# rasd3/3D-Dual-Fusion

Hardware: AMD Instinct MI355X
Metric: nuScenes sweeps/sec (0.075 m voxel, ~60k pts) (higher is better)
Workload: dtype f32 (fp32-grade throughout: every matrix-core GEMM -- C>=32 sparse convs, neck / head convs, FFN, query linears, image projection, value GEMM -- takes its fp32 operands as fp16 hi+lo pairs, 22 significand bits, 3 MFMA products, fp32 accumulate: <= 4e-6 of scale against float64, the grade of the exac

## Files before the change

### 3d-dual-fusion_amd/csrc/headconv.hip

```cpp
#include "common.h"
#include <algorithm>

namespace df3d {

typedef float f32x4 __attribute__((ext_vector_type(4)));
typedef unsigned int u32x4 __attribute__((ext_vector_type(4)));

constexpr int HF_TILE = 8, HF_HALO = HF_TILE + 2, HF_HP = HF_HALO * HF_HALO, HF_C = 64, HF_KMAX = 4;
constexpr int HF_LD = HF_HP + 1;

struct HeadFinalArgs {
  const u32x4 *in;
  const float *w;
  const u32x4 *wp;
  const float *bias;
  const int32_t *cols;
  float *out;
  int ld, ldo, B, H, W, G, tiles_x, tiles_y, gpad;
};

DF3D_SPLIT_OVERFLOW_TU(headconv)

__global__ __launch_bounds__(256) void head_final_kernel(HeadFinalArgs a) {
  __shared__ float x[HF_C * HF_LD];
// ... 274 lines not shown
        const int dy = tap / 3, dx = tap - dy * 3;
        const float *xp = x + lane * HF_LD + dy * HF_HALO + dx;
        for (int p = 0; p < 64; ++p) {
          const float xv = xp[(p >> 3) * HF_HALO + (p & 7)];
          const f32x4 g4 = *(const f32x4 *)&go[p * HF_KMAX];
          acc[i][0] = fmaf(xv, g4[0], acc[i][0]);
          acc[i][1] = fmaf(xv, g4[1], acc[i][1]);
          acc[i][2] = fmaf(xv, g4[2], acc[i][2]);
          acc[i][3] = fmaf(xv, g4[3], acc[i][3]);
        }
      }
    }
  }
#pragma unroll
  for (int i = 0; i < 3; ++i) {
    const int tap = wave + 4 * i;
    if (tap < 9) {
      float *dst = a.gw + (((size_t)g * 9 + tap) * HF_C + lane) * HF_KMAX;
#pragma unroll
      for (int j = 0; j < HF_KMAX; ++j)
        if (j < k && acc[i][j] != 0.f) unsafeAtomicAdd(dst + j, acc[i][j]);
    }
  }
}

}

using namespace df3d;

extern "C" size_t df3d_head_final_packed_bytes(int groups) { return groups > 0 ? (size_t)groups * 6 * 128 * 16 : 0; }

extern "C" int df3d_head_final_pack(const float *weights, int groups, void *packed, void *stream_) {
  hipStream_t stream = (hipStream_t)stream_;
  DF3D_CHECK_ARG(weights && packed && groups >= 1, "head_final_pack: bad argument");
  hipLaunchKernelGGL(head_final_pack_kernel, dim3(groups * 6), dim3(64), 0, stream, weights, (u32x4 *)packed);
  DF3D_LAUNCH_CHECK();
  return DF3D_OK;
}

static int head_final_impl(const void *in_split, int in_channels, int batch, int H, int W, int groups, const float *weights,
                           const void *packed, const float *bias, const int32_t *out_cols, float *out, int out_channels,
                           void *stream_);

extern "C" int df3d_head_final_conv(const void *in_split, int in_channels, int batch, int H, int W, int groups,
                                    const float *weights, const float *bias, const int32_t *out_cols, float *out,
                                    int out_channels, void *stream_) {
// ... 53 lines not shown
                                             const int32_t *out_cols, float *grad_acts, float *grad_weights, void *stream_) {
  hipStream_t stream = (hipStream_t)stream_;
  DF3D_CHECK_ARG(grad_out && weights && out_cols && (grad_acts || grad_weights), "head_final_conv_backward: null argument");
  DF3D_CHECK_ARG(groups >= 1 && act_channels >= groups * HF_C && act_channels % 4 == 0,
                 "head_final_conv_backward: %d branches of 64 channels do not fit %d-channel rows", groups, act_channels);
  DF3D_CHECK_ARG(batch >= 1 && H >= 1 && W >= 1 && out_channels >= 1, "head_final_conv_backward: bad sizes");
  DF3D_CHECK_ARG(!grad_weights || acts, "head_final_conv_backward: the filter gradient needs the activations");
  HeadFinalBwdArgs a;
  a.m = acts, a.go = grad_out, a.w = weights, a.cols = out_cols, a.gm = grad_acts, a.gw = grad_weights;
  a.ldm = act_channels, a.ldo = out_channels, a.B = batch, a.H = H, a.W = W, a.G = groups;
  a.tiles_x = cdiv(W, HF_TILE), a.tiles_y = cdiv(H, HF_TILE);
  const int ntiles = batch * a.tiles_x * a.tiles_y;
  a.tiles_per_wg = 1;
  if (grad_acts)
    hipLaunchKernelGGL(head_final_bwd_data_kernel, dim3(ntiles, groups), dim3(256), 0, stream, a);
  if (grad_weights) {
    DF3D_HIP(hipMemsetAsync(grad_weights, 0, (size_t)groups * 9 * HF_C * HF_KMAX * sizeof(float), stream));
    a.tiles_per_wg = std::max(1, cdiv(ntiles, 64));
    hipLaunchKernelGGL(head_final_bwd_filter_kernel, dim3(cdiv(ntiles, a.tiles_per_wg), groups), dim3(256), 0, stream, a);
  }
  DF3D_LAUNCH_CHECK();
  return DF3D_OK;
}
```

### 3d-dual-fusion_amd/dualfusion/_lib.py

```python
import ctypes
import os

_HERE = os.path.dirname(os.path.abspath(__file__))
LIB_PATH = os.path.join(os.path.dirname(_HERE), "csrc", "libdf3d_hip.so")

c_int = ctypes.c_int
c_uint = ctypes.c_uint
c_longlong = ctypes.c_longlong
c_size_t = ctypes.c_size_t
c_float = ctypes.c_float
c_void_p = ctypes.c_void_p
c_ulonglong = ctypes.c_ulonglong
c_char_p = ctypes.c_char_p

SIGNATURES = {
    "df3d_version": (c_int, []),
    "df3d_last_error": (c_char_p, []),
    "df3d_device_count": (c_int, []),
    "df3d_device_arch": (c_int, [c_char_p, c_int]),
    "df3d_split_overflow": (c_int, [c_int, c_char_p, c_int]),
    "df3d_split_overflow_collect": (c_int, [c_void_p, c_int, c_void_p]),
    "df3d_split_overflow_units": (c_int, [c_char_p, c_int]),
    "df3d_hard_voxelize_workspace_bytes": (c_size_t, [c_int, c_int, c_int]),
    "df3d_hard_voxelize": (c_int, [c_void_p, c_int, c_int, c_void_p, c_void_p, c_int, c_int, c_int,
# ... 130 lines not shown
    "df3d_sparse_conv_grad_filters": (c_int, [c_void_p, c_int, c_int, c_void_p, c_int, c_int, c_void_p, c_int, c_void_p,
                                              c_void_p]),
    "df3d_conv_rows_split": (c_int, [c_void_p, c_int, c_int, c_int, c_int, c_void_p, c_int, c_int, c_int, c_void_p, c_int,
                                     c_void_p, c_void_p, c_void_p, c_int, c_void_p, c_int, c_void_p, c_void_p, c_void_p]),
    "df3d_conv_packed_weight_bytes3": (c_size_t, [c_int, c_int, c_int]),
    "df3d_conv_pack_weights3": (c_int, [c_void_p, c_int, c_int, c_int, c_int, c_void_p, c_void_p]),
    "df3d_split_rows3": (c_int, [c_void_p, ctypes.c_longlong, c_int, c_void_p, c_void_p]),
    "df3d_conv_rows_split3": (c_int, [c_void_p, c_int, c_int, c_int, c_int, c_void_p, c_int, c_int, c_int, c_void_p, c_int,
                                      c_void_p, c_void_p, c_void_p, c_void_p, c_int, c_void_p, c_int, c_void_p, c_void_p,
                                      c_void_p]),
    "df3d_boxes_bev_pairwise": (c_int, [c_void_p, c_int, c_void_p, c_int, c_int, c_void_p, c_void_p]),
    "df3d_nms_bev_workspace_bytes": (c_size_t, [c_int, c_int]),
    "df3d_nms_bev": (c_int, [c_void_p, c_void_p, c_int, c_int, c_float, c_int, c_int, c_void_p, c_void_p, c_void_p,
                             c_size_t, c_void_p]),
    "df3d_centerhead_predict_workspace_bytes": (c_size_t, [c_int, c_void_p]),
    "df3d_centerhead_predict": (c_int, [c_void_p, c_int, c_void_p, c_void_p, c_void_p, c_void_p, c_void_p, c_void_p,
                                        c_size_t, c_void_p]),
    "df3d_head_final_conv": (c_int, [c_void_p, c_int, c_int, c_int, c_int, c_int, c_void_p, c_void_p, c_void_p, c_void_p,
                                     c_int, c_void_p]),
    "df3d_head_final_packed_bytes": (c_size_t, [c_int]),
    "df3d_head_final_pack": (c_int, [c_void_p, c_int, c_void_p, c_void_p]),
    "df3d_head_final_conv_packed": (c_int, [c_void_p, c_int, c_int, c_int, c_int, c_int, c_void_p, c_void_p, c_void_p,
                                            c_void_p, c_int, c_void_p]),
    "df3d_head_final_conv_backward": (c_int, [c_void_p, c_int, c_void_p, c_int, c_int, c_int, c_int, c_int, c_void_p, c_void_p,
                                              c_void_p, c_void_p, c_void_p]),
    "df3d_centerhead_loss_workspace_bytes": (c_size_t, [c_int, c_int, c_int, c_int]),
    "df3d_centerhead_loss": (c_int, [c_void_p, c_void_p, c_int, c_int, c_int, c_int, c_int, c_int, c_void_p, c_int, c_float,
                                     c_void_p, c_void_p, c_size_t, c_void_p]),
    "df3d_centerhead_loss_grad": (c_int, [c_void_p, c_void_p, c_void_p, c_int, c_int, c_int, c_int, c_int, c_int, c_void_p, c_int, c_float,
                                     c_void_p, c_void_p, c_size_t, c_void_p]),
    "df3d_heatmap_proposals_workspace_bytes": (c_size_t, [c_int, c_int, c_int, c_int]),
    "df3d_heatmap_proposals": (c_int, [c_void_p, c_int, c_int, c_int, c_int, c_int, c_int, c_uint, c_int, c_void_p, c_int,
                                       c_int, c_void_p, c_void_p, c_void_p, c_void_p, c_void_p, c_void_p, c_void_p,
                                       c_void_p, c_size_t, c_void_p]),
    "df3d_transfusion_decode": (c_int, [c_void_p, c_void_p, c_void_p, c_int, c_int, c_int, c_void_p, c_void_p, c_void_p,
                                        c_void_p, c_void_p, c_void_p]),
    "df3d_furthest_point_sample_with_dist": (c_int, [c_void_p, c_int, c_int, c_int, c_void_p, c_void_p, c_void_p]),
    "df3d_group_points_grad": (c_int, [c_void_p, c_void_p, c_int, c_int, c_int, c_int, c_int, c_void_p, c_void_p]),
    "df3d_gather_points_grad": (c_int, [c_void_p, c_void_p, c_int, c_int, c_int, c_int, c_void_p, c_void_p]),
    "df3d_rows_linear_packed_bytes": (c_size_t, [c_int, c_int]),
    "df3d_rows_linear": (c_int, [c_void_p, c_void_p, c_void_p, c_longlong, c_int, c_void_p, c_int, c_int, c_void_p, c_void_p, c_int,
                                 c_int, c_void_p, c_int, c_int, c_void_p, c_void_p, c_void_p, c_float, c_void_p]),
    "df3d_voxel_image_sample": (c_int, [c_void_p, c_int, c_int, c_float, c_void_p, c_void_p, c_void_p, c_void_p, c_void_p, c_int, c_int,
                                        c_int, c_int, c_int, c_float, c_float, c_void_p, c_void_p, c_void_p, c_void_p, c_void_p,
                                        c_void_p]),
    "df3d_backbone_inputs_ready": (c_int, [c_void_p]),
# ... 133 lines not shown
```

### 3d-dual-fusion_amd/dualfusion/apitimer.py

```python
import ctypes

from . import _lib

_NO_STREAM = ("df3d_version", "df3d_last_error", "df3d_device_count", "df3d_device_arch", "df3d_timing_", "df3d_ffn_set_precision",
              "df3d_conv_tile_count", "df3d_bn_rows_supported", "df3d_bn_rows_scratch_doubles", "df3d_debug_")
CONV_ENTRIES = ("df3d_sparse_conv_fused", "df3d_sparse_conv_grouped", "df3d_sparse_conv_fused_tiled", "df3d_sparse_conv_split", "df3d_sparse_conv_bf16",
                "df3d_conv_rows_split", "df3d_backbone_run")


def _ops_stream():
    from . import ops
    return ops._stream()


def _ival(a):
    if isinstance(a, bool):
        return int(a)
    if isinstance(a, int):
        return a
    if isinstance(a, (ctypes.c_int, ctypes.c_longlong, ctypes.c_size_t, ctypes.c_uint)):
        return int(a.value)
    if isinstance(a, float):
        return a
    if isinstance(a, ctypes.c_float):
# ... 101 lines not shown
    return B * ncam * max_ne * (C + Ci + 5) * 4, 0, "hbm", "gather of %d x %d query slots: %d voxel + %d image channels" % (B * ncam, max_ne, C, Ci)


def _rows(elems_in, elems_out, what):
    return (elems_in + elems_out) * 4, 0, "hbm", what


MODELS = {
    "df3d_hard_voxelize": lambda a, x: (20 * a[1] + a[6] * 0, 0, "hbm", "hash + scan + gather of %d points (bytes completed by the caller with M * 36)" % a[1]),
    "df3d_hard_voxelize_batched": lambda a, x: (20 * a[1], 0, "hbm", "hash + scan + gather of %d points (bytes completed by the caller with M * 36)" % a[1]),
    "df3d_ms_deform_attn_fused": lambda a, x: _msda(a, 4),
    "df3d_ms_deform_attn_fused_bf16": lambda a, x: _msda(a, 2),
    "df3d_ffn_fused_jobs": lambda a, x: _ffn(a, x),
    "df3d_imgproj_split": lambda a, x: _imgproj(a),
    "df3d_value_fold_gemm": lambda a, x: _value_gemm(a, 4),
    "df3d_value_fold_gemm_bf16": lambda a, x: _value_gemm(a, 2),
    "df3d_assemble_queries2": lambda a, x: _assemble(a),
    "df3d_sparse_to_dense": lambda a, x: (a[2] * a[3] * 4, 0, "hbm", "dense(): %d rows x %d channels scattered (+ the zero fill of the dense tensor)" % (a[2], a[3])),
    "df3d_sparse_to_dense_rows": lambda a, x: (a[2] * a[3] * 4, 0, "hbm", "dense() as pixel rows: %d rows x %d channels (+ the zero fill)" % (a[2], a[3])),
    "df3d_head_final_conv": lambda a, x: (a[2] * a[3] * a[4] * (a[1] * 4 + a[10] * 4), 2 * a[2] * a[3] * a[4] * a[5] * 9 * 64 * 4, "hbm",
                                          "final 3x3 convs of %d head branches on %d pixels" % (a[5], a[2] * a[3] * a[4])),
    "df3d_head_final_conv_packed": lambda a, x: (a[2] * a[3] * a[4] * (a[1] * 4 + a[10] * 4), 2 * a[2] * a[3] * a[4] * a[5] * 9 * 64 * 4, "hbm",
                                                 "final 3x3 convs of %d head branches on %d pixels (taps as matrix-core columns)" % (a[5], a[2] * a[3] * a[4])),
    "df3d_split_rows": lambda a, x: _rows(a[1] * a[2], a[1] * a[2], "fp32 rows -> split rows (%d x %d)" % (a[1], a[2])),
    "df3d_actr_prep": lambda a, x: _rows(3 * a[3] * a[4], 2 * a[3] * a[4], "query + position sums (%d rows)" % a[3]),
    "df3d_add_layernorm": lambda a, x: _rows(2 * a[5] * a[6], a[5] * a[6], "add + LayerNorm (%d rows)" % a[5]),
    "df3d_add_layernorm_split": lambda a, x: _rows(2 * a[5] * a[6], 2 * a[5] * a[6], "add + LayerNorm + split rows (%d rows)" % a[5]),
    "df3d_bigate_sum": lambda a, x: _rows(2 * a[6] * a[7], 2 * a[6] * a[7], "bidirectional gate (%d rows)" % a[6]),
    "df3d_rows_groupnorm": lambda a, x: _rows(2 * a[1] * a[2] * a[3], a[1] * a[2] * a[3], "GroupNorm over query rows (two passes)"),
    "df3d_fusion_writeback": lambda a, x: _rows(a[5] * a[6] + a[7] * a[8] * a[6], a[5] * a[6], "additive write-back of %d voxels" % a[5]),
    "df3d_rows_linear": lambda a, x: (a[3] * (a[4] + a[6]) * 4 + a[4] * a[6] * 4, 2 * a[3] * a[4] * a[6], "hbm",
                                      "query linear %d -> %d over %d rows (one input stream counted)" % (a[4], a[6], a[3])),
    "df3d_lt_layer": lambda a, x: (2 * a[1] * a[2] * a[3] * 4, a[1] * a[2] * 2 * (3 * 64 * 64 + 64 * 64 + 2 * 128 * 64 + 2 * 32 * 64), "hbm",
                                   "LocalTransformer layer over %d groups of %d tokens" % (a[2], a[1])),
    "df3d_lt_layer_gather": lambda a, x: (2 * 32 * a[3] * 64 * 4 + 32 * a[3] * 20, 32 * a[3] * 2 * (3 * 64 * 64 + 64 * 64 + 2 * 128 * 64 + 2 * 32 * 64 + 32 * 64), "hbm",
                                          "LocalTransformer layer with gather + positional MLP, %d groups" % a[3]),
    "df3d_lt_layer_scatter": lambda a, x: (2 * 32 * a[1] * 64 * 4 + 32 * a[1] * 8, 32 * a[1] * 2 * (3 * 64 * 64 + 64 * 64 + 2 * 128 * 64 + 2 * 32 * 64), "hbm",
                                           "LocalTransformer layer with winner write-back, %d groups" % a[1]),
    "df3d_voxel_image_sample": lambda a, x: (a[1] * (16 + a[9] * 4 * 5), 0, "hbm", "point-fusion sampling of %d voxels x %d channels" % (a[1], a[9])),
    "df3d_project_voxels": lambda a, x: (a[1] * 16 + a[1] * a[3] * (8 + 1 + 12 + 4), 0, "hbm", "projection of %d voxels into %d cameras" % (a[1], a[3])),
    "df3d_query_slots": lambda a, x: (a[2] * a[4] * 5 + a[2] * 16, 0, "hbm", "per-camera query slots of %d voxels" % a[2]),
}
RULEBOOK_ENTRIES = ("df3d_grid_build", "df3d_subm_neighbors", "df3d_conv_out_indices", "df3d_conv_neighbors",
                    "df3d_conv_transpose_out_indices", "df3d_conv_transpose_neighbors", "df3d_conv2d_neighbors", "df3d_nbr_to_pairs",
                    "df3d_pairs_to_nbr", "df3d_invert_neighbors")

# ... 30 lines not shown
```

### 3d-dual-fusion_amd/dualfusion/heads.py

```python
import copy
import os

import torch
from torch import nn

from . import ops as _ops
from .registry import HEADS


def _clamped_sigmoid(x):
    return torch.clamp(x.sigmoid_(), min=1e-4, max=1 - 1e-4)


def _transpose_and_gather_feat(feat, ind):
    feat = feat.permute(0, 2, 3, 1).contiguous()
    feat = feat.view(feat.size(0), -1, feat.size(3))
    return feat.gather(1, ind.unsqueeze(2).expand(ind.size(0), ind.size(1), feat.size(2)))


def reg_loss(output, mask, ind, target):
    pred = _transpose_and_gather_feat(output, ind)
    mask = mask.float().unsqueeze(2)
    loss = torch.nn.functional.l1_loss(pred * mask, target * mask, reduction='none')
    loss = loss / (mask.sum() + 1e-4)
# ... 69 lines not shown
        go = grad_out.contiguous().float()
        g_a, g_w = _ops.head_final_conv_backward(acts, go, B, H, W, w4d.shape[0], w4d, cols)
        sums = torch.cat([go.sum(0), go.new_zeros(1)])
        c = cols.long()
        j = torch.arange(4, device=go.device)
        idx = torch.where(j[None, :] < c[:, 1:2], c[:, 0:1] + j[None, :], torch.full_like(c[:, 0:1], go.shape[1]))
        return g_a, g_w, sums[idx], None, None, None, None, None


class _PermuteGather(torch.autograd.Function):

    @staticmethod
    def forward(ctx, src, idx, inv):
        ctx.save_for_backward(inv)
        return src.index_select(0, idx)

    @staticmethod
    @torch.autograd.function.once_differentiable
    def backward(ctx, grad):
        inv, = ctx.saved_tensors
        g = grad.contiguous().index_select(0, inv)
        g[-1] = 0
        return g, None, None


class SepHead(nn.Module):
    def __init__(self, in_channels, heads, head_conv=64, final_kernel=1, bn=False, init_bias=-2.19, **kwargs):
        super(SepHead, self).__init__(**kwargs)
        self.heads = heads
        for head in self.heads:
            classes, num_conv = self.heads[head]
            mods = []
            for _ in range(num_conv - 1):
                mods.append(nn.Conv2d(in_channels, head_conv, kernel_size=final_kernel, stride=1,
                                      padding=final_kernel // 2, bias=True))
                if bn:
                    mods.append(nn.BatchNorm2d(head_conv))
                mods.append(nn.ReLU())
            mods.append(nn.Conv2d(head_conv, classes, kernel_size=final_kernel, stride=1, padding=final_kernel // 2,
                                  bias=True))
            fc = nn.Sequential(*mods)
            if 'hm' in head:
                fc[-1].bias.data.fill_(init_bias)
            else:
                for m in fc.modules():
                    if isinstance(m, nn.Conv2d):
# ... 203 lines not shown
        _, s1 = _ops.conv_rows_split(split, 512, 0, plan["shared"], 64, 1, nbr, n, plan["s_bias"], plan["s_scale"],
                                     plan["s_shift"], relu=True, want_out=False, want_split=True)
        _, s2 = _ops.conv_rows_split(s1, 64, 0, plan["mid"], 64 * plan["mid_pair"], G // plan["mid_pair"], nbr, n,
                                     plan["mid_bias"], plan["mid_scale"], plan["mid_shift"], relu=True, want_out=False,
                                     want_split=True)
        if (plan["fin_w4"] is not None and os.environ.get("DF3D_HEAD_FINAL", "valu") == "valu"
                and _ops.CONV_PRECISION != "split3"):
            if "fin_pk" not in plan:
                plan["fin_pk"] = (_ops.head_final_pack(plan["fin_w4"])
                                  if os.environ.get("DF3D_HEADFINAL", "mfma")[:1] != "v" else None)
            out = _ops.head_final_conv(s2, B, H, W, plan["fin_w4"], plan["fin_b4"], plan["cols"], plan["width"],
                                       packed=plan["fin_pk"])
        else:
            out, _ = _ops.conv_rows_split(s2, 64, 64, plan["fin"], 32, G, nbr, n, plan["fin_bias"], None, None, relu=False,
                                          out_channels=plan["width"], out_cols=plan["cols"])
        rets = [dict() for _ in self.tasks]
        for t, head, c0, k in plan["layout"]:
            r = out[:, c0:c0 + k]
            v = r.view(B, H, W, k).permute(0, 3, 1, 2)
            v._df3d_rows = (r, None, v._version)
            rets[t][head] = v
        return rets

    def _final_pack(self, branches, dev):
        key = (tuple(fc[3].out_channels for _, _, fc in branches), str(dev))
        hit = self.__dict__.get("_final_pack_cache")
        if hit is not None and hit["key"] == key:
            return hit
        widx, bidx, cols, layout = [], [], [], []
        wbase = bbase = c0 = 0
        for _, _, fc in branches:
            k = fc[3].out_channels
            assert k <= 4 and fc[3].in_channels == 64 and fc[3].kernel_size == (3, 3)
            j, c, tap = torch.meshgrid(torch.arange(4), torch.arange(64), torch.arange(9), indexing="ij")
            idx = wbase + (j * 64 + c) * 9 + tap
            idx = torch.where(j < k, idx, torch.full_like(idx, -1))
            widx.append(idx.permute(2, 1, 0))
            bidx.append(torch.tensor([bbase + jj if jj < k else -1 for jj in range(4)]))
            cols.append((c0, k))
            layout.append((c0, k))
            wbase += k * 64 * 9
            bbase += k
            c0 += k
        widx = torch.stack(widx)
        bidx = torch.stack(bidx)
        widx[widx < 0] = wbase
# ... 102 lines not shown
                ret['auxseg_loss'] = auxseg_loss
                loss = loss + auxseg_loss
            keep = (lambda v: v.detach().cpu()) if host_copies else (lambda v: v.detach())
            ret.update({'loss': loss, 'hm_loss': keep(hm_loss), 'loc_loss': loc_loss,
                        'loc_loss_elem': keep(box_loss), 'num_positive': example['mask'][task_id].float().sum()})
            rets.append(ret)
        merged = defaultdict(list)
        for ret in rets:
            for k, v in ret.items():
                merged[k].append(v)
        return merged

    @torch.no_grad()
    def loss_device(self, example, preds_dicts):
        if self.dataset not in ('waymo', 'nuscenes'):
            raise NotImplementedError()
        B, _, H, W = preds_dicts[0]['hm'].shape
        tasks = []
        for pd in preds_dicts:
            d = {k: self._rows(pd[k]) for k in ('hm', 'reg', 'height', 'dim', 'rot')}
            if 'vel' in pd:
                d['vel'] = self._rows(pd['vel'])
            tasks.append(d)
        targets = [dict(hm=example['hm'][t], ind=example['ind'][t], mask=example['mask'][t], cat=example['cat'][t],
                        anno_box=example['anno_box'][t]) for t in range(len(preds_dicts))]
        ncodes = 10 if 'vel' in preds_dicts[0] else 8
        if len(self.code_weights) != ncodes:
            raise ValueError("code_weights has %d entries, the head regresses %d codes" % (len(self.code_weights), ncodes))
        out = _ops.centerhead_loss(tasks, targets, B, H, W, self.code_weights, self.weight)
        return {'loss': out[:, 0], 'hm_loss': out[:, 1], 'loc_loss': out[:, 2], 'num_positive': out[:, 3],
                'loc_loss_elem': out[:, 4:4 + ncodes]}

    @staticmethod
    def _rows(v):
        cached = getattr(v, "_df3d_rows", None)
        if cached is not None and cached[2] == v._version and cached[0].dtype == torch.float32:
            return cached[0]
        B, C, H, W = v.shape
        return v.float().permute(0, 2, 3, 1).reshape(B * H * W, C)

    @torch.no_grad()
    def predict_device(self, preds_dicts, test_cfg):
        get = test_cfg.get if hasattr(test_cfg, "get") else lambda k, d=None: getattr(test_cfg, k, d)
        if get('double_flip', False):
            raise NotImplementedError("double-flip test-time augmentation is not served by the device tail")
        if get('per_class_nms', False):
            raise NotImplementedError("per_class_nms is a no-op in the reference (center_head.py:431-432)")
        nms = get('nms')
        nms_get = nms.get if hasattr(nms, "get") else lambda k, d=None: getattr(nms, k, d)
# ... 43 lines not shown
```

### 3d-dual-fusion_amd/dualfusion/ops.py

```python
import collections
import ctypes
import os

import torch

from . import _lib


_raw_stream = getattr(torch._C, "_cuda_getCurrentRawStream", None)


def _stream():
    if _raw_stream is not None:
        return _lib.StreamArg(_raw_stream(torch.cuda.current_device()))
    return _lib.StreamArg(torch.cuda.current_stream().cuda_stream)


def _ptr(t):
    if t is None:
        return ctypes.c_void_p(0)
    rec = _lib._recorder
    if rec is not None:
        rec._tape.keep.append(t)
    return ctypes.c_void_p(t.data_ptr())
# ... 752 lines not shown
            raise _lib.Df3dError("conv_rows_split: columns [%d, %d) outside %d-channel rows" % (col0, col0 + groups * cout, oc))
        po = ctypes.c_void_p(out.data_ptr() + 4 * col0) if out is not None else None
        ps = ctypes.c_void_p(osp.data_ptr() + pb * col0) if osp is not None else None
        launch(po, oc, None, ps)
        return out, osp
    oc = int(out_channels if out_channels is not None else groups * cout)
    out = torch.empty((n_out, oc), dtype=torch.float32, device=dev) if want_out else None
    osp = torch.empty((n_out, pb * oc), dtype=torch.uint8, device=dev) if want_split else None
    launch(_ptr(out), oc, _ptr(out_cols), _ptr(osp))
    return out, osp


def head_final_pack(weights):
    lib = _lib.load()
    _chk(weights, torch.float32, "weights")
    G = weights.shape[0]
    if tuple(weights.shape[1:]) != (9, 64, 4):
        raise _lib.Df3dError("head_final_pack: weights [G,9,64,4] expected")
    packed = torch.empty(int(lib.df3d_head_final_packed_bytes(G)), dtype=torch.uint8, device=weights.device)
    _lib.check(lib.df3d_head_final_pack(_ptr(weights), G, _ptr(packed), _stream()), "df3d_head_final_pack")
    return packed


def head_final_conv(in_split, batch, H, W, weights, bias, out_cols, out_channels, packed=None):
    lib = _lib.load()
    _chk(in_split, torch.uint8, "in_split")
    _chk(weights, torch.float32, "weights")
    _chk(bias, torch.float32, "bias")
    _chk(out_cols, torch.int32, "out_cols")
    G = weights.shape[0]
    if tuple(weights.shape[1:]) != (9, 64, 4) or tuple(bias.shape) != (G, 4) or tuple(out_cols.shape) != (G, 2):
        raise _lib.Df3dError("head_final_conv: weights [G,9,64,4], bias [G,4], out_cols [G,2] expected")
    n = int(batch) * int(H) * int(W)
    if in_split.shape[0] != n:
        raise _lib.Df3dError("head_final_conv: %d rows for a %dx%dx%d map" % (in_split.shape[0], batch, H, W))
    out = torch.empty((n, int(out_channels)), dtype=torch.float32, device=in_split.device)
    if packed is not None:
        _chk(packed, torch.uint8, "packed")
        if packed.numel() != lib.df3d_head_final_packed_bytes(G):
            raise _lib.Df3dError("head_final_conv: packed filters do not match %d branches" % G)
        rc = lib.df3d_head_final_conv_packed(_ptr(in_split), in_split.shape[1] // 4, int(batch), int(H), int(W), G,
                                             _ptr(packed), _ptr(bias), _ptr(out_cols), _ptr(out), int(out_channels),
                                             _stream())
        _lib.check(rc, "df3d_head_final_conv_packed")
        return out
    rc = lib.df3d_head_final_conv(_ptr(in_split), in_split.shape[1] // 4, int(batch), int(H), int(W), G, _ptr(weights),
                                  _ptr(bias), _ptr(out_cols), _ptr(out), int(out_channels), _stream())
    _lib.check(rc, "df3d_head_final_conv")
    return out


def sparse_to_dense(features, indices, batch, shape):
    lib = _lib.load()
    _chk(features, torch.float32, "features")
    _chk(indices, torch.int32, "indices")
    n, C = features.shape
    out = torch.empty([int(batch), C] + [int(s) for s in shape], dtype=torch.float32, device=features.device)
    shp_p, keep = _lib.int3(shape)
    rc = lib.df3d_sparse_to_dense(_ptr(features), _ptr(indices), n, C, int(batch), shp_p, _ptr(out), _stream())
    _lib.check(rc, "df3d_sparse_to_dense")
    return out


def sparse_to_dense_rows(features, indices, batch, shape):
    lib = _lib.load()
    _chk(features, torch.float32, "features")
    _chk(indices, torch.int32, "indices")
    n, C = features.shape
    D, H, W = [int(v) for v in shape]
    out = torch.empty((int(batch) * H * W, C * D), dtype=torch.float32, device=features.device)
    shp_p, keep = _lib.int3(shape)
# ... 1584 lines not shown
```

### 3d-dual-fusion_amd/dualfusion/pipeline.py

```python
import os

import torch
from torch import nn

from . import synth
from .backbones import SpMiddleResNetFHD, SpMiddleResNetFHDFusion
from .voxel import Voxelization


class CenterPointHotPath(nn.Module):

    def __init__(self, fusion=None, voxel_size=synth.NUSC_VOXEL, pc_range=synth.NUSC_RANGE, max_points=10,
                 max_voxels=(120000, 160000), num_input_features=5, neck=None):
        super(CenterPointHotPath, self).__init__()
        self.voxel_layer = Voxelization(voxel_size, pc_range, max_points, max_voxels)
        if fusion is None:
            self.backbone = SpMiddleResNetFHD(num_input_features=num_input_features)
        else:
            self.backbone = SpMiddleResNetFHDFusion(num_input_features=num_input_features)
        self.fusion = fusion
        self.resident_inputs = False
        self.defer_neck = False
        self.neck = neck
        if neck is not None:
# ... 178 lines not shown
    launch_tape = os.environ.get("DF3D_LAUNCH_TAPE", "0") == "1"

    def train(self, mode=True):
        tape = self.__dict__.get("_tail_tape")
        if tape is not None:
            tape.reset()
        self.__dict__.pop("_tape_tensors", None)
        return super(CenterPointDetector, self).train(mode)

    def _tail_versions(self):
        ts = self.__dict__.get("_tape_tensors")
        if ts is None:
            mods = (self.hot_path.neck, self.bbox_head)
            ts = self.__dict__["_tape_tensors"] = [t for m in mods for t in list(m.parameters()) + list(m.buffers())]
        v = 0
        for t in ts:
            v += t._version
        return v

    def _neck_head(self, bev):
        rows, (nb, _, h, w) = bev
        return self.bbox_head(self.hot_path.neck.forward_rows(rows, nb, h, w))

    def _taped_tail(self, bev):
        from . import ops as _ops
        from .necks import SplitRows
        from .tape import TapedSection
        rows, (nb, c, h, w) = bev
        inp = rows.split if isinstance(rows, SplitRows) else rows
        tape = self.__dict__.get("_tail_tape")
        if tape is None:
            tape = self.__dict__["_tail_tape"] = TapedSection()
        key = (nb, c, h, w, tuple(inp.shape), inp.dtype, _ops.CONV_PRECISION, self._tail_versions(),
               os.environ.get("DF3D_HEAD_FINAL"), os.environ.get("DF3D_HEADFINAL"))
        return tape.run(key, lambda: self._neck_head(bev), [inp], _ops._stream())

    @torch.no_grad()
    def simple_test(self, points_list, batch_dict=None, example=None):
        from . import ops as _ops

        def run():
            preds = self._predictions(points_list, batch_dict, example)
            return self.bbox_head.predict(example if example is not None else {}, preds, self.test_cfg)
        return _ops.with_range_fallback(run)

    def _predictions(self, points_list, batch_dict=None, example=None):
        hp = self.hot_path
        taped = (self.launch_tape and not self.training and hp.neck is not None and hasattr(hp.neck, "forward_rows")
                 and getattr(hp.backbone, "dense_layout", "nchw") == "rows")
        hp.defer_neck = taped
        try:
            x, _ = hp(points_list, batch_dict=batch_dict, example=example)
        finally:
            hp.defer_neck = False
        return self._taped_tail(x) if taped else self.bbox_head(x)

    @torch.no_grad()
    def forward(self, points_list, batch_dict=None, example=None, return_loss=True):
        hp = self.hot_path
        taped = (self.launch_tape and not self.training and hp.neck is not None and hasattr(hp.neck, "forward_rows")
                 and getattr(hp.backbone, "dense_layout", "nchw") == "rows")
        hp.defer_neck = taped
        try:
            x, _ = hp(points_list, batch_dict=batch_dict, example=example)
        finally:
            hp.defer_neck = False
        preds = self._taped_tail(x) if taped else self.bbox_head(x)
        if return_loss:
            return self.bbox_head.loss_device(example, preds)
        return self.bbox_head.predict_device(preds, self.test_cfg)
```

### include/df3d_hip.h

```cpp
#ifndef DF3D_HIP_H_
#define DF3D_HIP_H_

#include <stddef.h>
#include <stdint.h>

#ifdef __cplusplus
extern "C" {
#endif

#define DF3D_OK 0
#define DF3D_EINVAL (-1)
#define DF3D_ENOMEM (-2)
#define DF3D_EHIP (-3)

#define DF3D_MAX_KVOL 32

int df3d_version(void);
const char *df3d_last_error(void);
int df3d_device_count(void);
int df3d_device_arch(char *buf, int buflen);
int df3d_split_overflow(int reset, char *where, int where_len);
int df3d_split_overflow_collect(uint32_t *out, int reset, void *stream);
int df3d_split_overflow_units(char *buf, int buflen);

// ... 147 lines not shown
} df3d_head_task;
typedef struct df3d_head_decode_cfg {
  int batch, H, W;
  float out_size_factor, voxel_size[2], pc_range[2];
  int has_post_center_range;
  float post_center_range[6];
  float score_threshold;
  int nms_mode;
  float nms_threshold;
  int pre_max, post_max;
} df3d_head_decode_cfg;
size_t df3d_centerhead_predict_workspace_bytes(int ntasks, const df3d_head_decode_cfg *cfg);
int df3d_centerhead_predict(const df3d_head_task *tasks, int ntasks, const df3d_head_decode_cfg *cfg, float *out_boxes,
                            float *out_scores, int32_t *out_labels, int32_t *out_counts, void *workspace,
                            size_t workspace_bytes, void *stream);

int df3d_head_final_conv(const void *in_split, int in_channels, int batch, int H, int W, int groups, const float *weights,
                         const float *bias, const int32_t *out_cols, float *out, int out_channels, void *stream);
size_t df3d_head_final_packed_bytes(int groups);
int df3d_head_final_pack(const float *weights, int groups, void *packed, void *stream);
int df3d_head_final_conv_packed(const void *in_split, int in_channels, int batch, int H, int W, int groups,
                                const void *packed, const float *bias, const int32_t *out_cols, float *out,
                                int out_channels, void *stream);
int df3d_head_final_conv_backward(const float *acts, int act_channels, const float *grad_out, int out_channels, int batch,
                                  int H, int W, int groups, const float *weights, const int32_t *out_cols,
                                  float *grad_acts, float *grad_weights, void *stream);

#define DF3D_LOSS_MAX_CODES 10
#define DF3D_LOSS_FIELDS (4 + DF3D_LOSS_MAX_CODES)
typedef struct df3d_head_targets {
  const float *hm;
  const long long *ind;
  const unsigned char *mask;
  const long long *cat;
  const float *box;
} df3d_head_targets;
size_t df3d_centerhead_loss_workspace_bytes(int ntasks, int batch, int H, int W);
int df3d_centerhead_loss(const df3d_head_task *tasks, const df3d_head_targets *targets, int ntasks, int batch, int H, int W,
                         int max_objs, int box_dim, const float *code_weights, int ncodes, float weight, float *out,
                         void *workspace, size_t workspace_bytes, void *stream);
int df3d_centerhead_loss_grad(const df3d_head_task *tasks, const df3d_head_task *grad_tasks, const df3d_head_targets *targets,
                              int ntasks, int batch, int H, int W, int max_objs, int box_dim, const float *code_weights,
                              int ncodes, float weight, float *out, void *workspace, size_t workspace_bytes, void *stream);

typedef struct df3d_query_heads {
  const float *heatmap, *center, *height, *dim, *rot, *vel;
// ... 373 lines not shown
```

Baseline: 370.9.

## Evaluate regression head branches only at target pixels in the eval-loss path

```diff
diff --git a/3d-dual-fusion_amd/csrc/headconv.hip b/3d-dual-fusion_amd/csrc/headconv.hip
--- a/3d-dual-fusion_amd/csrc/headconv.hip
+++ b/3d-dual-fusion_amd/csrc/headconv.hip
@@ -320,6 +320,139 @@
         if (j < k && acc[i][j] != 0.f) unsafeAtomicAdd(dst + j, acc[i][j]);
     }
   }
+}
+
+
+constexpr int HA_MAX_TASKS = 16;
+struct HeadAtArgs {
+  const u32x4 *s1;
+  const u32x4 *wmid;
+  const float *mbias, *mscale, *mshift;
+  const u32x4 *wfin;
+  const float *fbias;
+  const int32_t *cols;
+  const long long *ind[HA_MAX_TASKS];
+  unsigned *claimed;
+  float *out;
+  int ldo, B, H, W, M, NB, words;
+};
+
+template <int NBLK>
+__global__ __launch_bounds__(256) void head_regress_at_kernel(HeadAtArgs a) {
+  constexpr int FP = NBLK * 2;
+  constexpr int RQ = NBLK * 2 * 16;
+  __shared__ u32x4 mid[16 * RQ];
+  __shared__ float dd[NBLK * 2][9][HF_KMAX];
+  __shared__ int s_go;
+  const int tid = threadIdx.x, lane = tid & 63, n = lane & 15, g = lane >> 4;
+  const int wave = __builtin_amdgcn_readfirstlane(tid >> 6);
+  const int t = blockIdx.y, slot = blockIdx.x;
+  const int hw = a.H * a.W;
+  const long long ind = a.ind[t][slot];
+  if (ind < 0 || ind >= hw) return;
+  const int b = slot / a.M;
+  const long long row = (long long)b * hw + ind;
+  if (tid == 0) {
+    const unsigned bit = 1u << (unsigned)(row & 31);
+    s_go = (atomicOr(a.claimed + (size_t)t * a.words + (size_t)(row >> 5), bit) & bit) == 0u;
+  }
+  __syncthreads();
+  if (!s_go) return;
+  const int py = (int)(ind / a.W), px = (int)(ind - (long long)py * a.W);
+
+  const int qy = py + n / 3 - 1, qx = px + n % 3 - 1;
+  const bool qin = n < 9 && qy >= 0 && qy < a.H && qx >= 0 && qx < a.W;
+  f32x4 acc[FP];
+#pragma unroll
+  for (int i = 0; i < FP; ++i) acc[i] = (f32x4){0.f, 0.f, 0.f, 0.f};
+#pragma unroll
+  for (int k = 0; k < 9; ++k) {
+    const int sy = qy + k / 3 - 1, sx = qx + k % 3 - 1;
+    const bool in = qin && sy >= 0 && sy < a.H && sx >= 0 && sx < a.W;
+    const u32x4 *src = a.s1 + ((size_t)((size_t)b * a.H + (in ? sy : 0)) * a.W + (in ? sx : 0)) * 16 + g * 2;
+#pragma unroll
+    for (int kb = 0; kb < 2; ++kb) {
+      u32x4 ah = (u32x4){0u, 0u, 0u, 0u}, al = ah;
+      if (in) {
+        ah = src[kb * 8];
+        al = src[kb * 8 + 1];
+      }
+#pragma unroll
+      for (int i = 0; i < FP; ++i) {
+        const int f = wave * FP + i, blk = f >> 3, ct = f & 7;
+        const u32x4 *wb = a.wmid + ((((size_t)t * NBLK + blk) * 9 + k) * 2 + kb) * 1024 + ct * 128 + lane;
+        const u32x4 bh = wb[0], bl = wb[64];
+        acc[i] = HM_MFMA(al, bh, acc[i]);
+        acc[i] = HM_MFMA(ah, bl, acc[i]);
+        acc[i] = HM_MFMA(ah, bh, acc[i]);
+      }
+    }
+  }
+  float amax = 0.f;
+#pragma unroll
+  for (int i = 0; i < FP; ++i) {
+    const int f = wave * FP + i, blk = f >> 3, ct = f & 7;
+    const int c = blk * 128 + n * 8 + ct;
+    const int cg = t * (NBLK * 128) + c;
+    const float bi = a.mbias[cg], sc = a.mscale[cg], sh = a.mshift[cg];
+    f32x4 v = acc[i];
+    v = (v * DF3D_ACC_UNSCALE + (f32x4){bi, bi, bi, bi}) * (f32x4){sc, sc, sc, sc} + (f32x4){sh, sh, sh, sh};
+    v[0] = fmaxf(v[0], 0.f);
+    v[1] = fmaxf(v[1], 0.f);
+    v[2] = fmaxf(v[2], 0.f);
+    v[3] = fmaxf(v[3], 0.f);
+    const int br = c >> 6, ch = c & 63;
+    unsigned short *base = (unsigned short *)mid + br * 128 + (ch >> 3) * 16 + (ch & 7);
+#pragma unroll
+    for (int r = 0; r < 4; ++r) {
+      const int q = 4 * g + r;
+      const int ry = py + q / 3 - 1, rx = px + q % 3 - 1;
+      unsigned hi = 0u, lo = 0u;
+      if (q < 9 && ry >= 0 && ry < a.H && rx >= 0 && rx < a.W && br < a.NB) {
+        amax = fmaxf(amax, __builtin_fabsf(v[r]));
+        split_pair_nc(v[r], 0.f, hi, lo);
+      }
+      base[q * (RQ * 8)] = (unsigned short)(hi & 0xffffu);
+      base[q * (RQ * 8) + 8] = (unsigned short)(lo & 0xffffu);
+    }
+  }
+  split_range_flag(amax);
+  __syncthreads();
+  for (int br = wave; br < a.NB; br += 4) {
+    const int gb = t * a.NB + br;
+    u32x4 ah[2], al[2];
+#pragma unroll
+    for (int s = 0; s < 2; ++s) {
+      ah[s] = mid[n * RQ + br * 16 + s * 8 + g * 2];
+      al[s] = mid[n * RQ + br * 16 + s * 8 + g * 2 + 1];
+    }
+#pragma unroll
+    for (int ct = 0; ct < 3; ++ct) {
+      f32x4 d = (f32x4){0.f, 0.f, 0.f, 0.f};
+#pragma unroll
+      for (int s = 0; s < 2; ++s) {
+        const u32x4 *q = a.wfin + ((size_t)(gb * 3 + ct) * 2 + s) * 128 + lane;
+        const u32x4 bh = q[0], bl = q[64];
+        d = HM_MFMA(al[s], bh, d);
+        d = HM_MFMA(ah[s], bl, d);
+        d = HM_MFMA(ah[s], bh, d);
+      }
+      const int col = 16 * ct + n, tap = col >> 2, j = col & 3;
+      if (col < HM_PS) {
+#pragma unroll
+        for (int r = 0; r < 4; ++r)
+          if (4 * g + r == tap) dd[br][tap][j] = d[r] * DF3D_ACC_UNSCALE;
+      }
+    }
+  }
+  __syncthreads();
+  if (tid >= a.NB * HF_KMAX) return;
+  const int br = tid >> 2, j = tid & 3, gb = t * a.NB + br;
+  if (j >= a.cols[2 * gb + 1]) return;
+  float sum = 0.f;
+#pragma unroll
+  for (int tap = 0; tap < 9; ++tap) sum += dd[br][tap][j];
+  a.out[(size_t)row * a.ldo + a.cols[2 * gb] + j] = sum + a.fbias[gb * HF_KMAX + j];
 }
 
 }
@@ -419,3 +552,48 @@
   DF3D_LAUNCH_CHECK();
   return DF3D_OK;
 }
+
+extern "C" size_t df3d_head_regress_at_workspace_bytes(int tasks, int batch, int H, int W) {
+  if (tasks < 1 || batch < 1 || H < 1 || W < 1) return 0;
+  return (size_t)tasks * (((size_t)batch * H * W + 31) / 32) * sizeof(unsigned);
+}
+
+extern "C" int df3d_head_regress_at(const void *shared_split, int batch, int H, int W, int tasks, int branches,
+                                    const void *mid_packed, const float *mid_bias, const float *mid_scale,
+                                    const float *mid_shift, const void *fin_packed, const float *fin_bias,
+                                    const int32_t *out_cols, const long long *const *pixels, int per_sample, float *out,
+                                    int out_channels, void *workspace, size_t workspace_bytes, void *stream_) {
+  hipStream_t stream = (hipStream_t)stream_;
+  DF3D_CHECK_ARG(shared_split && mid_packed && mid_bias && mid_scale && mid_shift && fin_packed && fin_bias && out_cols &&
+                     pixels && out && workspace,
+                 "head_regress_at: null argument");
+  DF3D_CHECK_ARG(batch >= 1 && H >= 1 && W >= 1 && out_channels >= 1 && per_sample >= 1, "head_regress_at: bad sizes");
+  DF3D_CHECK_ARG((long long)batch * H * W <= 0x7fffffffLL, "head_regress_at: map too large");
+  DF3D_CHECK_ARG(tasks >= 1 && tasks <= HA_MAX_TASKS, "head_regress_at: 1 .. %d tasks, got %d", HA_MAX_TASKS, tasks);
+  DF3D_CHECK_ARG(branches >= 1 && branches <= 6, "head_regress_at: 1 .. 6 branches per task, got %d", branches);
+  DF3D_CHECK_ARG((long long)batch * per_sample <= 0x7fffffffLL && tasks <= 65535, "head_regress_at: too many slots");
+  const size_t need = df3d_head_regress_at_workspace_bytes(tasks, batch, H, W);
+  DF3D_CHECK_ARG(workspace_bytes >= need, "head_regress_at: workspace of %zu bytes, %zu needed", workspace_bytes, need);
+  HeadAtArgs a;
+  a.s1 = (const u32x4 *)shared_split;
+  a.wmid = (const u32x4 *)mid_packed;
+  a.mbias = mid_bias, a.mscale = mid_scale, a.mshift = mid_shift;
+  a.wfin = (const u32x4 *)fin_packed;
+  a.fbias = fin_bias;
+  a.cols = out_cols;
+  for (int t = 0; t < HA_MAX_TASKS; ++t) a.ind[t] = t < tasks ? pixels[t] : nullptr;
+  for (int t = 0; t < tasks; ++t) DF3D_CHECK_ARG(a.ind[t], "head_regress_at: null pixel list of task %d", t);
+  a.claimed = (unsigned *)workspace;
+  a.out = out;
+  a.ldo = out_channels;
+  a.B = batch, a.H = H, a.W = W, a.M = per_sample, a.NB = branches;
+  a.words = (int)(need / sizeof(unsigned) / tasks);
+  DF3D_HIP(hipMemsetAsync(workspace, 0, need, stream));
+  const dim3 grid((unsigned)(batch * per_sample), (unsigned)tasks);
+  const int nblk = (branches + 1) / 2;
+  if (nblk == 1) hipLaunchKernelGGL(head_regress_at_kernel<1>, grid, dim3(256), 0, stream, a);
+  else if (nblk == 2) hipLaunchKernelGGL(head_regress_at_kernel<2>, grid, dim3(256), 0, stream, a);
+  else hipLaunchKernelGGL(head_regress_at_kernel<3>, grid, dim3(256), 0, stream, a);
+  DF3D_LAUNCH_CHECK();
+  return DF3D_OK;
+}
diff --git a/3d-dual-fusion_amd/dualfusion/_lib.py b/3d-dual-fusion_amd/dualfusion/_lib.py
--- a/3d-dual-fusion_amd/dualfusion/_lib.py
+++ b/3d-dual-fusion_amd/dualfusion/_lib.py
@@ -176,6 +176,10 @@
     "df3d_head_final_pack": (c_int, [c_void_p, c_int, c_void_p, c_void_p]),
     "df3d_head_final_conv_packed": (c_int, [c_void_p, c_int, c_int, c_int, c_int, c_int, c_void_p, c_void_p, c_void_p,
                                             c_void_p, c_int, c_void_p]),
+    "df3d_head_regress_at_workspace_bytes": (c_size_t, [c_int, c_int, c_int, c_int]),
+    "df3d_head_regress_at": (c_int, [c_void_p, c_int, c_int, c_int, c_int, c_int, c_void_p, c_void_p, c_void_p, c_void_p,
+                                     c_void_p, c_void_p, c_void_p, c_void_p, c_int, c_void_p, c_int, c_void_p, c_size_t,
+                                     c_void_p]),
     "df3d_head_final_conv_backward": (c_int, [c_void_p, c_int, c_void_p, c_int, c_int, c_int, c_int, c_int, c_void_p, c_void_p,
                                               c_void_p, c_void_p, c_void_p]),
     "df3d_centerhead_loss_workspace_bytes": (c_size_t, [c_int, c_int, c_int, c_int]),
diff --git a/3d-dual-fusion_amd/dualfusion/apitimer.py b/3d-dual-fusion_amd/dualfusion/apitimer.py
--- a/3d-dual-fusion_amd/dualfusion/apitimer.py
+++ b/3d-dual-fusion_amd/dualfusion/apitimer.py
@@ -147,6 +147,7 @@
                                           "final 3x3 convs of %d head branches on %d pixels" % (a[5], a[2] * a[3] * a[4])),
     "df3d_head_final_conv_packed": lambda a, x: (a[2] * a[3] * a[4] * (a[1] * 4 + a[10] * 4), 2 * a[2] * a[3] * a[4] * a[5] * 9 * 64 * 4, "hbm",
                                                  "final 3x3 convs of %d head branches on %d pixels (taps as matrix-core columns)" % (a[5], a[2] * a[3] * a[4])),
+    "df3d_head_regress_at": lambda a, x: (None, None, "mfma", "regression branches of %d tasks x %d branches at <= %d listed pixels each (the claimed pixels are known on the device only)" % (a[4], a[5], a[1] * a[14])),
     "df3d_split_rows": lambda a, x: _rows(a[1] * a[2], a[1] * a[2], "fp32 rows -> split rows (%d x %d)" % (a[1], a[2])),
     "df3d_actr_prep": lambda a, x: _rows(3 * a[3] * a[4], 2 * a[3] * a[4], "query + position sums (%d rows)" % a[3]),
     "df3d_add_layernorm": lambda a, x: _rows(2 * a[5] * a[6], a[5] * a[6], "add + LayerNorm (%d rows)" % a[5]),
diff --git a/3d-dual-fusion_amd/dualfusion/heads.py b/3d-dual-fusion_amd/dualfusion/heads.py
--- a/3d-dual-fusion_amd/dualfusion/heads.py
+++ b/3d-dual-fusion_amd/dualfusion/heads.py
@@ -115,6 +115,12 @@
         g = grad.contiguous().index_select(0, inv)
         g[-1] = 0
         return g, None, None
+
+
+def lazy_loss_path(training, grad_enabled, dataset, precision, has_plan, env=None):
+    env = os.environ if env is None else env
+    return bool(not training and not grad_enabled and dataset in ('nuscenes', 'waymo') and precision == "split"
+                and has_plan and env.get("DF3D_HEAD_LAZY", "1") != "0")
 
 
 class SepHead(nn.Module):
@@ -364,6 +370,94 @@
             rets[t][head] = v
         return rets
 
+    def _lazy_plan(self):
+        plan = self._plan()
+        if "lazy" in plan:
+            return plan["lazy"]
+        plan["lazy"] = None
+        T = len(self.tasks)
+        names = [list(task.heads) for task in self.tasks]
+        reg = [h for h in names[0] if h != 'hm']
+        if (plan["fin_w4"] is None or set(reg) - {'vel'} != {'reg', 'height', 'dim', 'rot'} or T > 16
+                or not all('hm' in n and [h for h in n if h != 'hm'] == reg for n in names)):
+            return None
+        dev = plan["cols"].device
+        idx = {(t, head): i for i, (t, head, _, _) in enumerate(plan["layout"])}
+        G, NB = plan["groups"], len(reg)
+        hm_i = torch.tensor([idx[(t, 'hm')] for t in range(T)], device=dev)
+        reg_i = torch.tensor([idx[(t, h)] for t in range(T) for h in reg], device=dev)
+        first = lambda t, h: self._filters(getattr(self.tasks[t], h)[0])
+        per_col = lambda v, i: v.view(G, 64)[i]
+        pair = 2 if T % 2 == 0 else 1
+        hm_mid = [_ops.conv_pack_weights(torch.cat([first(t, 'hm') for t in range(i, i + pair)], dim=2).contiguous())
+                  for i in range(0, T, pair)]
+        nblk = (NB + 1) // 2
+        reg_mid = []
+        for t in range(T):
+            w = torch.cat([first(t, h) for h in reg] + [torch.zeros(9, 64, 64, device=dev)] * (2 * nblk - NB), dim=2)
+            reg_mid += [_ops.conv_pack_weights(w[:, :, i * 128:(i + 1) * 128].contiguous()) for i in range(nblk)]
+        padded = lambda v: torch.cat([per_col(v, reg_i).reshape(T, NB * 64),
+                                      torch.zeros(T, (2 * nblk - NB) * 64, device=dev)], 1).contiguous()
+        lazy = dict(pair=pair, hm_mid=torch.cat(hm_mid), hm_bias=per_col(plan["mid_bias"], hm_i).reshape(-1).contiguous(),
+                    hm_scale=per_col(plan["mid_scale"], hm_i).reshape(-1).contiguous(),
+                    hm_shift=per_col(plan["mid_shift"], hm_i).reshape(-1).contiguous(),
+                    hm_w4=plan["fin_w4"][hm_i].contiguous(), hm_b4=plan["fin_b4"][hm_i].contiguous(),
+                    hm_cols=plan["cols"][hm_i].contiguous(),
+                    branches=NB, reg_mid=torch.cat(reg_mid), reg_bias=padded(plan["mid_bias"]),
+                    reg_scale=padded(plan["mid_scale"]), reg_shift=padded(plan["mid_shift"]),
+                    reg_b4=plan["fin_b4"][reg_i].contiguous(), reg_cols=plan["cols"][reg_i].contiguous())
+        lazy["hm_pk"] = _ops.head_final_pack(lazy["hm_w4"])
+        lazy["reg_pk"] = _ops.head_final_pack(plan["fin_w4"][reg_i].contiguous())
+        plan["lazy"] = lazy
+        return lazy
+
+    def lazy_loss_applies(self, x=None, example=None):
+        w = self.shared_conv[0].weight
+        fits = (w.is_cuda and w.dtype == torch.float32 and (x is None or (x.is_cuda and x.dtype == torch.float32))
+                and example is not None and all(k in example for k in ('hm', 'ind', 'mask', 'cat', 'anno_box'))
+                and os.environ.get("DF3D_HEAD_FINAL", "valu") == "valu"
+                and os.environ.get("DF3D_HEADFINAL", "mfma")[:1] != "v")
+        if not lazy_loss_path(self.training, torch.is_grad_enabled(), self.dataset, _ops.CONV_PRECISION, fits):
+            return False
+        return self._row_kernels_fit(x) and self._lazy_plan() is not None
+
+    @torch.no_grad()
+    def forward_hm_rows(self, x, out=None):
+        from .necks import _rows_of
+        plan, lazy = self._plan(), self._lazy_plan()
+        B, _, H, W = x.shape
+        rows, split = _rows_of(x)
+        if (split is None or split.dtype != torch.uint8
+                or split.shape[1] != _ops.split_width(rows.shape[1])):
+            split = _ops.split_rows(rows.contiguous())
+        if (B, H, W) not in plan["nbr"]:
+            plan["nbr"][(B, H, W)] = _ops.conv2d_neighbors(B, H, W, 3, 3, 1, 1, False, x.device)[0]
+        nbr = plan["nbr"][(B, H, W)]
+        n = B * H * W
+        T = len(self.tasks)
+        _, s1 = _ops.conv_rows_split(split, 512, 0, plan["shared"], 64, 1, nbr, n, plan["s_bias"], plan["s_scale"],
+                                     plan["s_shift"], relu=True, want_out=False, want_split=True)
+        _, s2 = _ops.conv_rows_split(s1, 64, 0, lazy["hm_mid"], 64 * lazy["pair"], T // lazy["pair"], nbr, n,
+                                     lazy["hm_bias"], lazy["hm_scale"], lazy["hm_shift"], relu=True, want_out=False,
+                                     want_split=True)
+        out = _ops.head_final_conv(s2, B, H, W, lazy["hm_w4"], lazy["hm_b4"], lazy["hm_cols"], plan["width"],
+                                   packed=lazy["hm_pk"], out=out)
+        return out, s1, (B, H, W), plan
+
+    @torch.no_grad()
+    def loss_at_targets(self, example, packed):
+        out, s1, (B, H, W), plan = packed
+        lazy = plan["lazy"]
+        T = len(self.tasks)
+        pixels = [example['ind'][t] if example['ind'][t].is_contiguous() else example['ind'][t].contiguous()
+                  for t in range(T)]
+        _ops.head_regress_at(s1, B, H, W, lazy["branches"], lazy["reg_mid"], lazy["reg_bias"], lazy["reg_scale"],
+                             lazy["reg_shift"], lazy["reg_pk"], lazy["reg_b4"], lazy["reg_cols"], pixels, out)
+        tasks = [dict() for _ in range(T)]
+        for t, head, c0, k in plan["layout"]:
+            tasks[t][head] = out[:, c0:c0 + k]
+        return self._loss_of_rows(example, tasks, B, H, W)
+
     def _final_pack(self, branches, dev):
         key = (tuple(fc[3].out_channels for _, _, fc in branches), str(dev))
         hit = self.__dict__.get("_final_pack_cache")
@@ -512,9 +606,12 @@
             if 'vel' in pd:
                 d['vel'] = self._rows(pd['vel'])
             tasks.append(d)
+        return self._loss_of_rows(example, tasks, B, H, W)
+
+    def _loss_of_rows(self, example, tasks, B, H, W):
         targets = [dict(hm=example['hm'][t], ind=example['ind'][t], mask=example['mask'][t], cat=example['cat'][t],
-                        anno_box=example['anno_box'][t]) for t in range(len(preds_dicts))]
-        ncodes = 10 if 'vel' in preds_dicts[0] else 8
+                        anno_box=example['anno_box'][t]) for t in range(len(tasks))]
+        ncodes = 10 if 'vel' in tasks[0] else 8
         if len(self.code_weights) != ncodes:
             raise ValueError("code_weights has %d entries, the head regresses %d codes" % (len(self.code_weights), ncodes))
         out = _ops.centerhead_loss(tasks, targets, B, H, W, self.code_weights, self.weight)
diff --git a/3d-dual-fusion_amd/dualfusion/ops.py b/3d-dual-fusion_amd/dualfusion/ops.py
--- a/3d-dual-fusion_amd/dualfusion/ops.py
+++ b/3d-dual-fusion_amd/dualfusion/ops.py
@@ -798,7 +798,7 @@
     return packed
 
 
-def head_final_conv(in_split, batch, H, W, weights, bias, out_cols, out_channels, packed=None):
+def head_final_conv(in_split, batch, H, W, weights, bias, out_cols, out_channels, packed=None, out=None):
     lib = _lib.load()
     _chk(in_split, torch.uint8, "in_split")
     _chk(weights, torch.float32, "weights")
@@ -810,7 +810,10 @@
     n = int(batch) * int(H) * int(W)
     if in_split.shape[0] != n:
         raise _lib.Df3dError("head_final_conv: %d rows for a %dx%dx%d map" % (in_split.shape[0], batch, H, W))
-    out = torch.empty((n, int(out_channels)), dtype=torch.float32, device=in_split.device)
+    if out is None:
+        out = torch.empty((n, int(out_channels)), dtype=torch.float32, device=in_split.device)
+    elif _chk(out, torch.float32, "out").shape != (n, int(out_channels)):
+        raise _lib.Df3dError("head_final_conv: out must be [%d, %d]" % (n, int(out_channels)))
     if packed is not None:
         _chk(packed, torch.uint8, "packed")
         if packed.numel() != lib.df3d_head_final_packed_bytes(G):
@@ -823,6 +826,44 @@
     rc = lib.df3d_head_final_conv(_ptr(in_split), in_split.shape[1] // 4, int(batch), int(H), int(W), G, _ptr(weights),
                                   _ptr(bias), _ptr(out_cols), _ptr(out), int(out_channels), _stream())
     _lib.check(rc, "df3d_head_final_conv")
+    return out
+
+
+def head_regress_at(shared_split, batch, H, W, branches, mid_packed, mid_bias, mid_scale, mid_shift, fin_packed, fin_bias,
+                    out_cols, pixels, out):
+    lib = _lib.load()
+    T = len(pixels)
+    nblk = (int(branches) + 1) // 2
+    n = int(batch) * int(H) * int(W)
+    _chk(shared_split, torch.uint8, "shared_split")
+    if tuple(shared_split.shape) != (n, 256):
+        raise _lib.Df3dError("head_regress_at: two-part split rows [%d, 64 channels] expected" % n)
+    _chk(mid_packed, torch.uint8, "mid_packed")
+    if mid_packed.numel() != T * nblk * 9 * 64 * 128 * 4:
+        raise _lib.Df3dError("head_regress_at: packed first convs do not match %d tasks x %d blocks" % (T, nblk))
+    for v, nm in ((mid_bias, "mid_bias"), (mid_scale, "mid_scale"), (mid_shift, "mid_shift")):
+        if _chk(v, torch.float32, nm).numel() != T * nblk * 128:
+            raise _lib.Df3dError("head_regress_at: %s must hold %d x %d columns" % (nm, T, nblk * 128))
+    _chk(fin_packed, torch.uint8, "fin_packed")
+    if fin_packed.numel() != lib.df3d_head_final_packed_bytes(T * int(branches)):
+        raise _lib.Df3dError("head_regress_at: packed final convs do not match %d branches" % (T * int(branches)))
+    if tuple(_chk(fin_bias, torch.float32, "fin_bias").shape) != (T * int(branches), 4) \
+            or tuple(_chk(out_cols, torch.int32, "out_cols").shape) != (T * int(branches), 2):
+        raise _lib.Df3dError("head_regress_at: fin_bias [T*branches, 4] and out_cols [T*branches, 2] expected")
+    if _chk(out, torch.float32, "out").dim() != 2 or out.shape[0] != n:
+        raise _lib.Df3dError("head_regress_at: out must be [%d, width]" % n)
+    M = int(pixels[0].shape[1])
+    for p in pixels:
+        if tuple(_chk(p, torch.int64, "pixels").shape) != (int(batch), M):
+            raise _lib.Df3dError("head_regress_at: every pixel list must be int64 [%d, %d]" % (int(batch), M))
+    ptrs = (ctypes.c_void_p * T)(*[p.data_ptr() for p in pixels])
+    nbytes = int(lib.df3d_head_regress_at_workspace_bytes(T, int(batch), int(H), int(W)))
+    ws = torch.empty((nbytes,), dtype=torch.uint8, device=out.device)
+    rc = lib.df3d_head_regress_at(_ptr(shared_split), int(batch), int(H), int(W), T, int(branches), _ptr(mid_packed),
+                                  _ptr(mid_bias), _ptr(mid_scale), _ptr(mid_shift), _ptr(fin_packed), _ptr(fin_bias),
+                                  _ptr(out_cols), ctypes.cast(ptrs, ctypes.c_void_p), M, _ptr(out), int(out.shape[1]),
+                                  _ptr(ws), nbytes, _stream())
+    _lib.check(rc, "df3d_head_regress_at")
     return out
 
 
diff --git a/3d-dual-fusion_amd/dualfusion/pipeline.py b/3d-dual-fusion_amd/dualfusion/pipeline.py
--- a/3d-dual-fusion_amd/dualfusion/pipeline.py
+++ b/3d-dual-fusion_amd/dualfusion/pipeline.py
@@ -224,7 +224,11 @@
         rows, (nb, _, h, w) = bev
         return self.bbox_head(self.hot_path.neck.forward_rows(rows, nb, h, w))
 
-    def _taped_tail(self, bev):
+    def _neck_head_hm(self, bev):
+        rows, (nb, _, h, w) = bev
+        return self.bbox_head.forward_hm_rows(self.hot_path.neck.forward_rows(rows, nb, h, w))
+
+    def _taped_tail(self, bev, lazy=False):
         from . import ops as _ops
         from .necks import SplitRows
         from .tape import TapedSection
@@ -234,8 +238,8 @@
         if tape is None:
             tape = self.__dict__["_tail_tape"] = TapedSection()
         key = (nb, c, h, w, tuple(inp.shape), inp.dtype, _ops.CONV_PRECISION, self._tail_versions(),
-               os.environ.get("DF3D_HEAD_FINAL"), os.environ.get("DF3D_HEADFINAL"))
-        return tape.run(key, lambda: self._neck_head(bev), [inp], _ops._stream())
+               os.environ.get("DF3D_HEAD_FINAL"), os.environ.get("DF3D_HEADFINAL"), bool(lazy))
+        return tape.run(key, lambda: (self._neck_head_hm if lazy else self._neck_head)(bev), [inp], _ops._stream())
 
     @torch.no_grad()
     def simple_test(self, points_list, batch_dict=None, example=None):
@@ -267,7 +271,12 @@
             x, _ = hp(points_list, batch_dict=batch_dict, example=example)
         finally:
             hp.defer_neck = False
-        preds = self._taped_tail(x) if taped else self.bbox_head(x)
+        head = self.bbox_head
+        if (return_loss and hasattr(head, "lazy_loss_applies")
+                and head.lazy_loss_applies(None if taped else x, example)):
+            packed = self._taped_tail(x, lazy=True) if taped else head.forward_hm_rows(x)
+            return head.loss_at_targets(example, packed)
+        preds = self._taped_tail(x) if taped else head(x)
         if return_loss:
-            return self.bbox_head.loss_device(example, preds)
-        return self.bbox_head.predict_device(preds, self.test_cfg)
+            return head.loss_device(example, preds)
+        return head.predict_device(preds, self.test_cfg)
diff --git a/include/df3d_hip.h b/include/df3d_hip.h
--- a/include/df3d_hip.h
+++ b/include/df3d_hip.h
@@ -193,6 +193,12 @@
 int df3d_head_final_conv_packed(const void *in_split, int in_channels, int batch, int H, int W, int groups,
                                 const void *packed, const float *bias, const int32_t *out_cols, float *out,
                                 int out_channels, void *stream);
+size_t df3d_head_regress_at_workspace_bytes(int tasks, int batch, int H, int W);
+int df3d_head_regress_at(const void *shared_split, int batch, int H, int W, int tasks, int branches,
+                         const void *mid_packed, const float *mid_bias, const float *mid_scale, const float *mid_shift,
+                         const void *fin_packed, const float *fin_bias, const int32_t *out_cols,
+                         const long long *const *pixels, int per_sample, float *out, int out_channels, void *workspace,
+                         size_t workspace_bytes, void *stream);
 int df3d_head_final_conv_backward(const float *acts, int act_channels, const float *grad_out, int out_channels, int batch,
                                   int H, int W, int groups, const float *weights, const int32_t *out_cols,
                                   float *grad_acts, float *grad_weights, void *stream);
```

Result: faster. 401.2 (median of 5 runs) (+8.2%).
